# E-J408/admm-net

Measured on AMD Instinct MI355X. Metric: signals/sec (K-layer ADMM-Net forward), higher is better.
Workload: dtype f32; 1 GPU; cfg3: ADMMNet K=16 grid 16x16 (D=256, n=257) batch 65536/GPU + spectrum on 1024 atoms; batch_per_gpu=65536, global_batch=65536, K=16, D=256, n=257, natoms=1024, batch_mean_scope=global, chunk=8192, weights=torch.manual_seed(0) default init, glayer=matrix function, checked per matrix; eigensolver on the rejected matrices

## Files before the change

admm_net_amd/csrc/spectral_fused.hip:

```cpp
#include <stdio.h>
#include <stdlib.h>

#include <type_traits>

#include "common.h"
#include "rebuild_core.h"
#include "lane_reduce.h"

namespace admmnet {

constexpr int SF_THREADS = 768, SF_WAVES = 12;
constexpr int SF_PITCH = 40;
constexpr int SF_MAXM = 4;

typedef __bf16 bf16x8 __attribute__((ext_vector_type(8)));
typedef __bf16 bf16x2 __attribute__((ext_vector_type(2)));
typedef float f32x2v __attribute__((ext_vector_type(2)));
using f32x16 = __attribute__((ext_vector_type(16))) float;

__device__ __forceinline__ unsigned sf_pack_bf16(float a, float b) {
    const f32x2v p = {a, b};
    return __builtin_bit_cast(unsigned, __builtin_convertvector(p, bf16x2));
}
__device__ __forceinline__ float sf_bf16_lo(unsigned u) { return __uint_as_float(u << 16); }
// ... 19 lines not shown
#pragma unroll
    for (int q = 0; q < 4; ++q) {
        float v = 0.f;
#pragma unroll
        for (int w = 0; w < W; ++w) v += red[q * W + w];
        s[q] = v;
    }
    a = s[0]; b = s[1]; c = s[2]; d = s[3];
}

template <int W>
__device__ __forceinline__ void sf_block_sum8(float &a, float &b, float &c, float &d, float &e, float &f, float *red ) {
    const float t = sf_reduce4(a, b, c, d), u = sf_reduce4(e, f, 0.f, 0.f);
    const int lane = threadIdx.x & 63, wave = threadIdx.x >> 6;
    __syncthreads();
    if ((lane & 15) == 0) {
        red[(lane >> 4) * W + wave] = t;
        red[(4 + (lane >> 4)) * W + wave] = u;
    }
    __syncthreads();
    float s[6];
#pragma unroll
    for (int q = 0; q < 6; ++q) {
        float v = 0.f;
#pragma unroll
        for (int w = 0; w < W; ++w) v += red[q * W + w];
        s[q] = v;
    }
    a = s[0]; b = s[1]; c = s[2]; d = s[3]; e = s[4]; f = s[5];
}

struct SfCarve {
    int NP, NJ;
    float2 *X0, *X1, *Y0, *Y1, *ph, *Ob;
    float *hh, *hp, *red, *coef;
    double *sc;
    int *flags;
    float2 *part;
    unsigned short *ETre;
    unsigned short *ETim;
    __host__ __device__ static int np_of(int n) { return (n + 7) & ~7; }
    __host__ __device__ static int nj_of(int n) {
        const int D = n - 1, nt = (D + 31) >> 5;
        const int a = 32 * nt, b = (n + 7) & ~7;
        return a > b ? a : b;
    }
    __host__ __device__ static size_t bytes(int n, int W) {
        const size_t NP = np_of(n), NJ = nj_of(n);
        const size_t fixed = sizeof(float2) * 6 * NP + sizeof(float) * 2 * NP + sizeof(float) * 96 + sizeof(float) * 16 +
                             sizeof(double) * 16 + sizeof(int) * 4;
        const size_t part = sizeof(float2) * W * 2 * NP;
        const size_t slab = sizeof(unsigned short) * 2 * NJ * SF_PITCH;
        return fixed + (part > slab ? part : slab) + 64;
    }
    __device__ SfCarve(char *smem, int n) {
        NP = np_of(n);
        NJ = nj_of(n);
        sc = reinterpret_cast<double *>(smem);
        X0 = reinterpret_cast<float2 *>(sc + 16);
        X1 = X0 + NP; Y0 = X1 + NP; Y1 = Y0 + NP; ph = Y1 + NP; Ob = ph + NP;
        hh = reinterpret_cast<float *>(Ob + NP);
        hp = hh + NP;
        red = hp + NP;
        coef = red + 96;
        flags = reinterpret_cast<int *>(coef + 16);
        const int fixed = (int)(sizeof(double) * 16 + sizeof(float2) * 6 * NP + sizeof(float) * 2 * NP + sizeof(float) * 112 +
                                sizeof(int) * 4);
        char *u = smem + ((fixed + 15) & ~15);
        part = reinterpret_cast<float2 *>(u);
        ETre = reinterpret_cast<unsigned short *>(u);
        ETim = ETre + NJ * SF_PITCH;
    }
};

struct SfUpdate {
    const float *alpha;
    const float2 *phi_prev;
    const float *h_prev;
    const float *lw_prev;
    int mode;
};

__device__ __forceinline__ float2 sf_a_elem(int i, int j, int D, float2 z, float ir, float corner, float hi, float2 phj) {
    float2 a = make_float2(-ir * z.x, -ir * z.y);
    if (i < D) {
        if (i == j) a = make_float2(hi - ir * z.x, 0.f);
    } else {
        a = (j == D) ? make_float2(corner - ir * z.x, 0.f) : make_float2(phj.x - ir * z.x, -phj.y - ir * z.y);
    }
    return a;
}

template <int TPW, int W>
__global__ __launch_bounds__(64 * W, W == 12 ? 1 : 3) void sp_fused_kernel(int D, const float *__restrict__ lw, const float2 *__restrict__ phi,
                                                                 const float *__restrict__ h, float2 *Zg,
                                                                 float2 *G, float *__restrict__ rn,
                                                                 int *__restrict__ flag, int32_t *__restrict__ status, float tol,
                                                                 int iters, unsigned long long *__restrict__ ptime, SfUpdate up) {
    extern __shared__ __attribute__((aligned(16))) char smem[];
    long long t_prev = ptime ? clock64() : 0;
    auto mark = [&](int id) {
        if (ptime && threadIdx.x == 0) {
            const long long t_now = clock64();
            atomicAdd(&ptime[id], (unsigned long long)(t_now - t_prev));
            t_prev = t_now;
        }
    };
    const int n = D + 1;
    const SfCarve cv(smem, n);
    const int NP = cv.NP;
    const int64_t b = blockIdx.x;
    float2 *Z = Zg + b * (int64_t)n * n;
    const float2 *Gold = G + b * (int64_t)n * n;
    const int tid = threadIdx.x, lane = tid & 63;
    const int wave = __builtin_amdgcn_readfirstlane(tid >> 6);
    const float ir = lw[S_INV_RHO_G], corner = lw[S_CORNER_G];
    const int NT = (D + 31) >> 5, ntri = NT * (NT + 1) / 2;
    const int MM = (n + 63) >> 6;

    float pn = 0.f;
    if (tid < NP) {
        const float2 p = tid < D ? phi[b * D + tid] : make_float2(0.f, 0.f);
        cv.ph[tid] = p;
        cv.hh[tid] = tid < D ? h[b * D + tid] : 0.f;
        pn = p.x * p.x + p.y * p.y;
        if (up.mode) {
            cv.Ob[tid] = tid < D ? up.phi_prev[b * D + tid] : make_float2(0.f, 0.f);
            cv.hp[tid] = tid < D ? up.h_prev[b * D + tid] : 0.f;
        }
    }
    const float al = up.mode ? up.alpha[b] : 0.f;
    const float corner_zp = up.mode ? up.lw_prev[S_CORNER_Z] : 0.f;
    {
        float z1 = 0.f, z2 = 0.f, z3 = 0.f;
        sf_block_sum4<W>(pn, z1, z2, z3, cv.red);
    }
    const float ipn = pn > 0.f ? rsqrtf(pn) : 0.f;
    if (tid < NP) {
        const float2 p = cv.ph[tid];
        cv.X0[tid] = make_float2(tid == D ? 1.f : 0.f, 0.f);
        cv.X1[tid] = pn > 0.f ? make_float2(p.x * ipn, p.y * ipn) : make_float2(tid == 0 ? 1.f : 0.f, 0.f);
    }
    __syncthreads();

    mark(0);
    double trace = 0.0;
    float l0 = 0.f, l1 = 0.f, cf = 0.f, res0 = 0.f, res1 = 0.f;
    bool last = false;
    for (int it = 0; it < iters; ++it) {
        v2f x0[SF_MAXM], x1[SF_MAXM], c0[SF_MAXM], c1[SF_MAXM];
#pragma unroll
        for (int m = 0; m < SF_MAXM; ++m) {
            const int j = lane + 64 * m;
            const bool v = m < MM && j < n;
            x0[m] = v ? pk2(cv.X0[j]) : v2f{0.f, 0.f};
            x1[m] = v ? pk2(cv.X1[j]) : v2f{0.f, 0.f};
            c0[m] = v2f{0.f, 0.f};
            c1[m] = v2f{0.f, 0.f};
        }
        float trl = 0.f;
        auto run_pass = [&](auto updc) {
        constexpr bool UPD = decltype(updc)::value;
        float2 za[SF_MAXM], zb[SF_MAXM], zc[SF_MAXM], zd[SF_MAXM];
        float2 ga[SF_MAXM], gb[SF_MAXM], gc[SF_MAXM], gd[SF_MAXM];
        auto load_row = [&](int i, float2(&z)[SF_MAXM], float2(&g)[SF_MAXM]) {
#pragma unroll
            for (int m = 0; m < SF_MAXM; ++m) {
                const int j = lane + 64 * m;
                const bool v = i < n && j <= i;
                z[m] = (v && !(UPD && up.mode == 2)) ? Z[(int64_t)i * n + j] : make_float2(0.f, 0.f);
                if (UPD) g[m] = v ? Gold[(int64_t)i * n + j] : make_float2(0.f, 0.f);
            }
        };
        auto proc_row = [&](int i, float2(&zc)[SF_MAXM], const float2(&gq)[SF_MAXM]) {
            if (UPD) {
                const float hpi = cv.hp[i];
#pragma unroll
                for (int m = 0; m < SF_MAXM; ++m) {
                    if (64 * m <= i) {
                        const int j = lane + 64 * m;
                        if (j <= i) {
                            float2 c;
                            if (i < D) c = make_float2(i == j ? hpi : 0.f, 0.f);
                            else if (j == D) c = make_float2(corner_zp, 0.f);
                            else {
                                const float2 pp = cv.Ob[j];
                                c = make_float2(pp.x, -pp.y);
                            }
                            const float2 zn = make_float2(zc[m].x + al * (gq[m].x - c.x), zc[m].y + al * (gq[m].y - c.y));
                            zc[m] = zn;
                            Z[(int64_t)i * n + j] = zn;
                        }
                    }
                }
            }
            const v2f xi0 = pk2(cv.X0[i]), xi1 = pk2(cv.X1[i]);
            const float hi = cv.hh[i];
            v2f r0 = {0.f, 0.f}, r1 = {0.f, 0.f};
#pragma unroll
            for (int m = 0; m < SF_MAXM; ++m) {
                if (64 * m <= i) {
                    const int j = lane + 64 * m;
                    float2 a = sf_a_elem(i, j, D, zc[m], ir, corner, hi, (i == D && j < D) ? cv.ph[j] : make_float2(0.f, 0.f));
                    if (j > i) a = make_float2(0.f, 0.f);
                    if (j == i) trl += a.x;
                    const v2f av = pk2(a);
                    r0 = pk_cfma(r0, av, x0[m]);
                    r1 = pk_cfma(r1, av, x1[m]);
                    const v2f ac = (j < i) ? av : v2f{0.f, 0.f};
                    c0[m] = pk_cfma_conj(c0[m], ac, xi0);
                    c1[m] = pk_cfma_conj(c1[m], ac, xi1);
                }
            }
            if (i == 64 * SF_MAXM && lane == 0) {
                const int64_t idx = (int64_t)i * n + i;
                float2 z = (UPD && up.mode == 2) ? make_float2(0.f, 0.f) : Z[idx];
                if (UPD) {
                    const float2 g = Gold[idx];
                    z = make_float2(z.x + al * (g.x - corner_zp), z.y + al * g.y);
                    Z[idx] = z;
                }
                const float a = corner - ir * z.x;
                trl += a;
                const float2 xa = cv.X0[i], xb = cv.X1[i];
                r0.x += a * xa.x; r0.y += a * xa.y;
                r1.x += a * xb.x; r1.y += a * xb.y;
            }
            const float t = sf_reduce4(r0.x, r0.y, r1.x, r1.y);
            if ((lane & 15) == 0) {
                float *dst = reinterpret_cast<float *>((lane & 32) ? cv.Y1 : cv.Y0);
                dst[2 * i + ((lane >> 4) & 1)] = t;
            }
        };
        load_row(wave, za, ga);
        load_row(wave + W, zb, gb);
        for (int i = wave; i < n; i += 2 * W) {
            load_row(i + 2 * W, zc, gc);
            load_row(i + 3 * W, zd, gd);
            proc_row(i, za, ga);
            if (i + W < n) proc_row(i + W, zb, gb);
#pragma unroll
            for (int m = 0; m < SF_MAXM; ++m) {
                za[m] = zc[m];
                zb[m] = zd[m];
                ga[m] = gc[m];
                gb[m] = gd[m];
            }
        }
        };
        if (up.mode != 0 && it == 0) run_pass(std::true_type{});
        else run_pass(std::false_type{});
#pragma unroll
        for (int m = 0; m < SF_MAXM; ++m) {
            const int j = lane + 64 * m;
            if (m < MM && j < NP) {
                cv.part[(wave * 2 + 0) * NP + j] = make_float2(c0[m].x, c0[m].y);
                cv.part[(wave * 2 + 1) * NP + j] = make_float2(c1[m].x, c1[m].y);
            }
        }
        if (it == 0) {
            float z1 = 0.f, z2 = 0.f, z3 = 0.f;
            sf_block_sum4<W>(trl, z1, z2, z3, cv.red);
            trace = (double)trl;
        }
        __syncthreads();
        mark(1);
        float2 x0e = make_float2(0.f, 0.f), x1e = x0e, y0e = x0e, y1e = x0e;
        if (tid < n) {
            y0e = cv.Y0[tid];
            y1e = cv.Y1[tid];
#pragma unroll
            for (int w = 0; w < W; ++w) {
                if (tid >= 64 * SF_MAXM) break;
                const float2 p0 = cv.part[(w * 2 + 0) * NP + tid], p1 = cv.part[(w * 2 + 1) * NP + tid];
                y0e.x += p0.x; y0e.y += p0.y;
                y1e.x += p1.x; y1e.y += p1.y;
            }
            x0e = cv.X0[tid];
            x1e = cv.X1[tid];
        }
        float h00 = x0e.x * y0e.x + x0e.y * y0e.y, h11 = x1e.x * y1e.x + x1e.y * y1e.y;
        float h01r = x0e.x * y1e.x + x0e.y * y1e.y, h01i = x0e.x * y1e.y - x0e.y * y1e.x;
        sf_block_sum4<W>(h00, h11, h01r, h01i, cv.red);
        float ct = 1.f, st = 0.f, er = 1.f, ei = 0.f;
        {
            const float ab = sqrtf(h01r * h01r + h01i * h01i);
            const float dif = 0.5f * (h00 - h11), rad = sqrtf(dif * dif + ab * ab);
            l0 = 0.5f * (h00 + h11) - rad;
            l1 = 0.5f * (h00 + h11) + rad;
            const float vx = dif >= 0.f ? dif + rad : ab, vy = dif >= 0.f ? ab : rad - dif;
            const float nrm = sqrtf(vx * vx + vy * vy);
            if (nrm > 0.f) {
                ct = vx / nrm;
                st = vy / nrm;
            }
            if (ab > 0.f) {
                er = h01r / ab;
                ei = -h01i / ab;
            }
            cf = (float)((trace - (double)l0 - (double)l1) / (double)(n - 2));
            if (tid == 0) {
                cv.sc[0] = l0; cv.sc[1] = l1; cv.sc[2] = cf;
            }
        }
        const float2 ex1 = make_float2(er * x1e.x - ei * x1e.y, er * x1e.y + ei * x1e.x);
        const float2 ey1 = make_float2(er * y1e.x - ei * y1e.y, er * y1e.y + ei * y1e.x);
        const float2 nx0 = make_float2(-st * x0e.x + ct * ex1.x, -st * x0e.y + ct * ex1.y);
        const float2 nx1 = make_float2(ct * x0e.x + st * ex1.x, ct * x0e.y + st * ex1.y);
        const float2 ny0 = make_float2(-st * y0e.x + ct * ey1.x, -st * y0e.y + ct * ey1.y);
        const float2 ny1 = make_float2(ct * y0e.x + st * ey1.x, ct * y0e.y + st * ey1.y);
        const float2 d0 = make_float2(ny0.x - l0 * nx0.x, ny0.y - l0 * nx0.y);
        const float2 d1 = make_float2(ny1.x - l1 * nx1.x, ny1.y - l1 * nx1.y);
        float r0s = d0.x * d0.x + d0.y * d0.y, r1s = d1.x * d1.x + d1.y * d1.y;
        const float2 p0 = make_float2(ny0.x - cf * nx0.x, ny0.y - cf * nx0.y);
        const float2 p1 = make_float2(ny1.x - cf * nx1.x, ny1.y - cf * nx1.y);
        float n0 = p0.x * p0.x + p0.y * p0.y, n1 = p1.x * p1.x + p1.y * p1.y;
        float pr = p0.x * p1.x + p0.y * p1.y, pi = p0.x * p1.y - p0.y * p1.x;
        sf_block_sum8<W>(r0s, r1s, n0, n1, pr, pi, cv.red);
        res0 = sqrtf(r0s);
        res1 = sqrtf(r1s);
        last = it + 1 >= iters ||
               (it >= 1 && res0 <= 2e-6f * fabsf(l0 - cf) && res1 <= 2e-6f * fabsf(l1 - cf));
        if (!last) {
            const float in0 = n0 > 0.f ? rsqrtf(n0) : 0.f;
            const float2 q0 = make_float2(p0.x * in0, p0.y * in0);
            const float gr = pr * in0, gi = pi * in0;
            float2 q1 = make_float2(p1.x - (gr * q0.x - gi * q0.y), p1.y - (gr * q0.y + gi * q0.x));
            const float n1o = n1 - (gr * gr + gi * gi);
            const float in1 = n1o > 0.f ? rsqrtf(n1o) : 0.f;
            q1.x *= in1;
            q1.y *= in1;
            if (tid < NP) {
                cv.X0[tid] = tid < n ? q0 : make_float2(0.f, 0.f);
                cv.X1[tid] = tid < n ? q1 : make_float2(0.f, 0.f);
            }
        } else if (tid < NP) {
            cv.X0[tid] = tid < n ? nx0 : make_float2(0.f, 0.f);
            cv.X1[tid] = tid < n ? nx1 : make_float2(0.f, 0.f);
        }
        __syncthreads();
        mark(2);
        if (last) break;
    }
    const float mu0 = l0 - cf, mu1 = l1 - cf;

    int tI[TPW], tJ[TPW];
#pragma unroll
    for (int s = 0; s < TPW; ++s) tri_tile(wave * TPW + s, tI[s], tJ[s]);
    f32x16 accRe[TPW], accIm[TPW];
#pragma unroll
    for (int s = 0; s < TPW; ++s) {
#pragma unroll
        for (int q = 0; q < 16; ++q) {
            accRe[s][q] = 0.f;
            accIm[s][q] = 0.f;
        }
    }
    float2 ob = make_float2(0.f, 0.f);
    unsigned *ETre32 = reinterpret_cast<unsigned *>(cv.ETre), *ETim32 = reinterpret_cast<unsigned *>(cv.ETim);
    constexpr int P32 = SF_PITCH / 2;
    for (int idx = tid; idx < (cv.NJ - n) * P32; idx += (64 * W)) {
        ETre32[n * P32 + idx] = 0u;
        ETim32[n * P32 + idx] = 0u;
    }
    const int nslab = (n + 31) >> 5;
    for (int K = 0; K < nslab; ++K) {
        const int k0 = 32 * K;
        __syncthreads();
        int tl = tid;
        asm volatile("" : "+v"(tl));
        auto deflate = [&](float2 a, float2 vr0, float2 vc0, float2 vr1, float2 vc1, bool diag) {
            const float2 q0 = cmulc(vr0, vc0), q1 = cmulc(vr1, vc1);
            a.x -= mu0 * q0.x + mu1 * q1.x;
            a.y -= mu0 * q0.y + mu1 * q1.y;
            if (diag) {
                a.x -= cf;
                a.y = 0.f;
            }
            return a;
        };
        auto pair_of = [&](const float2 *v, int k, float2 &lo, float2 &hi) {
            const float4 t = *reinterpret_cast<const float4 *>(v + k);
            lo = make_float2(t.x, t.y);
            hi = make_float2(t.z, t.w);
        };
        {
            constexpr int RP = (64 * W) / 256, LQ = (16 + RP - 1) / RP;
            const int j = tl & 255;
            const float2 vj0 = cv.X0[j], vj1 = cv.X1[j], phj = cv.ph[j];
            constexpr int LB = 3;
// ... 98 lines not shown
                        accIm[s] = __builtin_amdgcn_mfma_f32_32x32x16_bf16(Are, Bim, accIm[s], 0, 0, 0);
                        accRe[s] = __builtin_amdgcn_mfma_f32_32x32x16_bf16(Aim, Bim, accRe[s], 0, 0, 0);
                        accIm[s] = __builtin_amdgcn_mfma_f32_32x32x16_bf16(Aim, nBre, accIm[s], 0, 0, 0);
                    }
                }
            }
        }
        mark(4);
        __syncthreads();
        if (tid < n) {
            const unsigned *dre = ETre32 + D * P32, *dim = ETim32 + D * P32;
            const unsigned *jre = ETre32 + tid * P32, *jim = ETim32 + tid * P32;
#pragma unroll 2
            for (int kp = 0; kp < 16; ++kp) {
                const unsigned ur = dre[kp], ui = dim[kp], vr = jre[kp], vi = jim[kp];
                const float ar0 = sf_bf16_lo(ur), ai0 = sf_bf16_lo(ui), br0 = sf_bf16_lo(vr), bi0 = sf_bf16_lo(vi);
                const float ar1 = sf_bf16_hi(ur), ai1 = sf_bf16_hi(ui), br1 = sf_bf16_hi(vr), bi1 = sf_bf16_hi(vi);
                {
                    asm volatile("v_fma_f32 %0, %1, %2, %0" : "+v"(ob.x) : "v"(ar0), "v"(br0));
                    asm volatile("v_fma_f32 %0, %1, %2, %0" : "+v"(ob.x) : "v"(ai0), "v"(bi0));
                    asm volatile("v_fma_f32 %0, %1, %2, %0" : "+v"(ob.x) : "v"(ar1), "v"(br1));
                    asm volatile("v_fma_f32 %0, %1, %2, %0" : "+v"(ob.x) : "v"(ai1), "v"(bi1));
                    asm volatile("v_fma_f32 %0, %1, %2, %0" : "+v"(ob.y) : "v"(ar0), "v"(bi0));
                    asm volatile("v_fma_f32 %0, -%1, %2, %0" : "+v"(ob.y) : "v"(ai0), "v"(br0));
                    asm volatile("v_fma_f32 %0, %1, %2, %0" : "+v"(ob.y) : "v"(ar1), "v"(bi1));
                    asm volatile("v_fma_f32 %0, -%1, %2, %0" : "+v"(ob.y) : "v"(ai1), "v"(br1));
                }
            }
        }
        mark(5);
    }
    __syncthreads();
    if (tid < NP) cv.Ob[tid] = tid < n ? ob : make_float2(0.f, 0.f);

    float fro = 0.f;
    {
        const int r32 = lane & 31, kh = lane >> 5;
#pragma unroll
        for (int s = 0; s < TPW; ++s) {
            if (wave * TPW + s < ntri) {
                const float wgt = tI[s] == tJ[s] ? 1.f : 2.f;
                const int gj = 32 * tJ[s] + r32;
#pragma unroll
                for (int q = 0; q < 16; ++q) {
                    const int gi = 32 * tI[s] + (q & 3) + 8 * (q >> 2) + 4 * kh;
                    if (gi < D && gj < D) fro += wgt * (accRe[s][q] * accRe[s][q] + accIm[s][q] * accIm[s][q]);
                }
            }
        }
        if (tid < n) fro += (tid < D ? 2.f : 1.f) * (ob.x * ob.x + ob.y * ob.y);
        float z1 = 0.f, z2 = 0.f, z3 = 0.f;
        sf_block_sum4<W>(fro, z1, z2, z3, cv.red);
    }
    const LayerLayout L{D};
    const float *vn = lw + L.off_vn();
    if (wave == 0) {
        const double thr = lw[S_THR];
        const double dl0 = cv.sc[0], dl1 = cv.sc[1], c = cv.sc[2];
        const double delta = sqrt(sqrt((double)fro)) * (1.0 + 0x1p-8);
        const double ts[9] = {-1.0, 0.0, 1.0, -0.75, -0.5, -0.25, 0.25, 0.5, 0.75};
        double arg = c;
        if (lane < 9) arg = c + ts[lane] * delta;
        else if (lane == 9) arg = dl0;
        else if (lane == 10) arg = dl1;
        const double fv = eig_map_f64(arg, thr, vn);
        auto bcast = [&](int src) {
            const long long bits = __builtin_bit_cast(long long, fv);
            const int lo = __builtin_amdgcn_readlane((int)(bits & 0xffffffffll), src);
            const int hi = __builtin_amdgcn_readlane((int)(bits >> 32), src);
            return __builtin_bit_cast(double, ((long long)hi << 32) | (unsigned long long)(unsigned)lo);
        };
        const double fm = bcast(0), fc = bcast(1), fp = bcast(2), f0k = bcast(9), f1k = bcast(10);
        const double a0 = fc, a1 = (fp - fm) / (2.0 * delta), a2 = (fp - 2.0 * fc + fm) / (2.0 * delta * delta);
        const double scale = fmax(fmax(fabs(fc), fmax(fabs(f0k), fabs(f1k))), 1e-6);
        double miss = 0.0;
        if (lane >= 3 && lane < 9) {
            const double t = ts[lane] * delta;
            miss = fabs(fv - (a0 + a1 * t + a2 * t * t));
        }
#pragma unroll
        for (int o = 8; o > 0; o >>= 1) miss = fmax(miss, __shfl_xor(miss, o, 64));
        if (lane == 0) {
            int why = 0;
            const double g0 = fabs(dl0 - c), g1 = fabs(dl1 - c);
            if (!(isfinite(dl0) && isfinite(dl1) && isfinite(c) && isfinite(delta) && delta > 0.0 && isfinite(miss))) why = 8;
            else if (!((double)res0 <= 1e-5 * fmax(g0, 1e-30) && (double)res1 <= 1e-5 * fmax(g1, 1e-30))) why = 1;
            else if (!(delta < 0.05 * fmin(g0, g1))) why = 2;
            else if (!(miss <= (double)tol * scale)) why = 4;
            else if (!(fabs(a2) * delta * delta <= 1e-4 * scale)) why = 16;
            cv.coef[0] = (float)(a0 - a1 * c);
            cv.coef[1] = (float)a1;
            cv.coef[2] = (float)a2;
            cv.coef[3] = (float)(f0k - a0 - a1 * (dl0 - c));
            cv.coef[4] = (float)(f1k - a0 - a1 * (dl1 - c));
            cv.flags[0] = why;
            flag[b] = why;
            if (status) {
                atomicAdd(status + (why ? 1 : 2), 1);
                if (why == 4) atomicAdd(status + 3, 1);
            }
        }
    }
    __syncthreads();
    mark(6);
    if (cv.flags[0]) return;

    const float k0c = cv.coef[0], a1f = cv.coef[1], a2f = cv.coef[2], g0f = cv.coef[3], g1f = cv.coef[4];
    const float corner_z = lw[S_CORNER_Z];
    float2 *Gb = G + b * (int64_t)n * n;
    float acc = 0.f;
    {
        const int r32 = lane & 31, kh = lane >> 5;
#pragma unroll
        for (int s = 0; s < TPW; ++s) {
            if (wave * TPW + s < ntri) {
                const int gj = 32 * tJ[s] + r32;
                const float2 vj0 = cv.X0[gj < n ? gj : 0], vj1 = cv.X1[gj < n ? gj : 0];
                constexpr int AB = 16;
#pragma unroll
                for (int qb = 0; qb < 16; qb += AB) {
                    float2 zq[AB];
#pragma unroll
                    for (int u = 0; u < AB; ++u) {
                        const int q = qb + u, gi = 32 * tI[s] + (q & 3) + 8 * (q >> 2) + 4 * kh;
                        zq[u] = (gi < D && gj <= gi) ? Z[(int64_t)gi * n + gj] : make_float2(0.f, 0.f);
                    }
#pragma unroll
                    for (int u = 0; u < AB; ++u) {
                        const int q = qb + u, gi = 32 * tI[s] + (q & 3) + 8 * (q >> 2) + 4 * kh;
                        if (gi < D && gj <= gi) {
                            const float hi = cv.hh[gi];
                            const float2 a = sf_a_elem(gi, gj, D, zq[u], ir, corner, hi, make_float2(0.f, 0.f));
                            const float2 p0 = cmulc(cv.X0[gi], vj0), p1 = cmulc(cv.X1[gi], vj1);
                            float2 g = make_float2(a1f * a.x + a2f * accRe[s][q] + g0f * p0.x + g1f * p1.x,
                                                   a1f * a.y + a2f * accIm[s][q] + g0f * p0.y + g1f * p1.y);
                            float cz = 0.f;
                            if (gi == gj) {
                                g.x += k0c;
                                g.y = 0.f;
                                cz = hi;
                            }
                            Gb[(int64_t)gi * n + gj] = g;
                            const float dr = g.x - cz;
                            acc += (gi == gj ? 1.f : 2.f) * (dr * dr + g.y * g.y);
                        }
                    }
                }
            }
        }
    }
    if (tid < n) {
        const int j = tid;
        const float2 a = sf_a_elem(D, j, D, Z[(int64_t)D * n + j], ir, corner, 0.f, cv.ph[j]);
        const float2 o = cv.Ob[j];
        const float2 p0 = cmulc(cv.X0[D], cv.X0[j]), p1 = cmulc(cv.X1[D], cv.X1[j]);
        float2 g = make_float2(a1f * a.x + a2f * o.x + g0f * p0.x + g1f * p1.x, a1f * a.y + a2f * o.y + g0f * p0.y + g1f * p1.y);
        float2 cz = make_float2(cv.ph[j].x, -cv.ph[j].y);
        if (j == D) {
            g.x += k0c;
            g.y = 0.f;
            cz = make_float2(corner_z, 0.f);
        }
        Gb[(int64_t)D * n + j] = g;
        const float dr = g.x - cz.x, di = g.y - cz.y;
        acc += (j == D ? 1.f : 2.f) * (dr * dr + di * di);
    }
    {
        float z1 = 0.f, z2 = 0.f, z3 = 0.f;
        sf_block_sum4<W>(acc, z1, z2, z3, cv.red);
    }
    if (tid == 0) rn[b] = sqrtf(acc);
    mark(7);
}

template <int TPW, int W>
static int sf_launch(int D, int64_t nb, const float *lw, const float2 *phi, const float *h, float2 *Z, float2 *G, float *rn,
                     int *flag, int32_t *status, float tol, int iters, bool timing, const SfUpdate &up, hipStream_t st) {
    const size_t lds = SfCarve::bytes(D + 1, W);
    ADMM_HIP(hipFuncSetAttribute(reinterpret_cast<const void *>(sp_fused_kernel<TPW, W>), hipFuncAttributeMaxDynamicSharedMemorySize,
                                 (int)lds));
    PhaseTimer tm;
    if (int rc = tm.begin(timing, st, 16)) return rc;
    hipLaunchKernelGGL((sp_fused_kernel<TPW, W>), dim3((unsigned)nb), dim3(64 * W), lds, st, D, lw, phi, h, Z, G, rn, flag, status,
                       tol, iters, tm.dev, up);
    ADMM_HIP(hipGetLastError());
    if (tm.dev) {
        unsigned long long hb[16];
        if (int rc = tm.end(st, hb)) return rc;
        fprintf(stderr, "[sf timing D=%d nb=%lld] cycles per workgroup: setup %.0f | matvec %.0f ritz %.0f (all passes) | stage %.0f "
                "mfma %.0f border %.0f (all slabs) | model %.0f | assemble %.0f\n", D, (long long)nb, hb[0] / (double)nb,
                hb[1] / (double)nb, hb[2] / (double)nb, (hb[3]) / (double)nb, hb[4] / (double)nb, hb[5] / (double)nb,
                hb[6] / (double)nb, hb[7] / (double)nb);
    }
    return ADMMNET_OK;
}

static_assert(SF_WAVES == 12, "spectral_waves (route.h) names the shapes 4 and 12");

int launch_spectral_fused(const Switches &sw, int D, int64_t nb, const float *lw, const float2 *phi, const float *h, float2 *Z,
                          float2 *G, float *rn, int *flag, int32_t *status, const float *alpha, const float2 *phi_prev,
                          const float *h_prev, const float *lw_prev, int update_mode, int waves, hipStream_t st) {
    const SfUpdate up{alpha, phi_prev, h_prev, lw_prev, update_mode};
    if (D < 2 || D > 256) {
        set_error("spectral: D=%d outside 2..256", D);
        return ADMMNET_E_ARG;
    }
    if (!(waves == SF_WAVES || (waves == 4 && D <= 128))) {
        set_error("spectral: %d waves per matrix at D=%d (need 12, or 4 with D <= 128)", waves, D);
        return ADMMNET_E_ARG;
    }
    const float tol = sw.spectral_tol;
    const int iters = sw.spectral_iters;
    const bool timing = sw.sf_timing;
    const int NT = (D + 31) >> 5, ntri = NT * (NT + 1) / 2;
    if (waves == 4) {
        switch ((ntri + 3) / 4) {
            case 1: return sf_launch<1, 4>(D, nb, lw, phi, h, Z, G, rn, flag, status, tol, iters, timing, up, st);
            case 2: return sf_launch<2, 4>(D, nb, lw, phi, h, Z, G, rn, flag, status, tol, iters, timing, up, st);
            default: return sf_launch<3, 4>(D, nb, lw, phi, h, Z, G, rn, flag, status, tol, iters, timing, up, st);
        }
    }
    switch ((ntri + SF_WAVES - 1) / SF_WAVES) {
        case 1: return sf_launch<1, SF_WAVES>(D, nb, lw, phi, h, Z, G, rn, flag, status, tol, iters, timing, up, st);
        case 2: return sf_launch<2, SF_WAVES>(D, nb, lw, phi, h, Z, G, rn, flag, status, tol, iters, timing, up, st);
        default: return sf_launch<3, SF_WAVES>(D, nb, lw, phi, h, Z, G, rn, flag, status, tol, iters, timing, up, st);
// ... 5 lines not shown
```

Baseline: 93960 signals/s.

## Fuse deflated-matrix staging into the last matvec pass with LDS-resident image

For the 12-wave shape, the last power/Ritz iteration now also writes a bf16 image of the deflated matrix (lower-triangle tiles plus a border strip) straight into LDS. The later MFMA spectral stage then reads that image instead of re-reading Z from global memory and re-staging it. A guard compares the predicted deflation against the final Ritz values and reruns the old path if the staged image is stale. The change adds LDS pressure (checked against a 160 KiB limit) and a serialized per-wave Y accumulation. It also adds a profiling summary script.

After: 107,200 signals/s, median of 6. 14.1% higher.

```diff
diff --git a/admm_net_amd/csrc/spectral_fused.hip b/admm_net_amd/csrc/spectral_fused.hip
--- a/admm_net_amd/csrc/spectral_fused.hip
+++ b/admm_net_amd/csrc/spectral_fused.hip
@@ -75,46 +75,70 @@
 
 struct SfCarve {
     int NP, NJ;
-    float2 *X0, *X1, *Y0, *Y1, *ph, *Ob;
+    float2 *X0, *X1, *Y0, *Y1, *ph, *Ob, *pp;
     float *hh, *hp, *red, *coef;
     double *sc;
     int *flags;
     float2 *part;
     unsigned short *ETre;
     unsigned short *ETim;
+    unsigned short *img;
+    unsigned *strip;
     __host__ __device__ static int np_of(int n) { return (n + 7) & ~7; }
     __host__ __device__ static int nj_of(int n) {
         const int D = n - 1, nt = (D + 31) >> 5;
         const int a = 32 * nt, b = (n + 7) & ~7;
         return a > b ? a : b;
     }
+    __host__ __device__ static constexpr bool resident(int W) { return W == SF_WAVES; }
+    __host__ __device__ static size_t img_bytes(int n) {
+        const size_t nt = (n - 1 + 31) >> 5;
+        return nt * (nt + 1) / 2 * 4096;
+    }
+    __host__ __device__ static size_t fixed_bytes(int n, int W) {
+        const size_t NP = np_of(n);
+        return sizeof(double) * 16 + sizeof(float2) * 6 * NP + sizeof(float) * (resident(W) ? 1 : 2) * NP + sizeof(float) * 112 +
+               sizeof(int) * 4;
+    }
     __host__ __device__ static size_t bytes(int n, int W) {
         const size_t NP = np_of(n), NJ = nj_of(n);
-        const size_t fixed = sizeof(float2) * 6 * NP + sizeof(float) * 2 * NP + sizeof(float) * 96 + sizeof(float) * 16 +
-                             sizeof(double) * 16 + sizeof(int) * 4;
         const size_t part = sizeof(float2) * W * 2 * NP;
+        if (resident(W)) {
+            const size_t a = part + sizeof(float) * 3 * NP, b = img_bytes(n) + sizeof(unsigned) * NJ;
+            return fixed_bytes(n, W) + (a > b ? a : b) + 64;
+        }
         const size_t slab = sizeof(unsigned short) * 2 * NJ * SF_PITCH;
-        return fixed + (part > slab ? part : slab) + 64;
-    }
-    __device__ SfCarve(char *smem, int n) {
+        return fixed_bytes(n, W) + (part > slab ? part : slab) + 64;
+    }
+    __device__ SfCarve(char *smem, int n, int W) {
         NP = np_of(n);
         NJ = nj_of(n);
         sc = reinterpret_cast<double *>(smem);
         X0 = reinterpret_cast<float2 *>(sc + 16);
         X1 = X0 + NP; Y0 = X1 + NP; Y1 = Y0 + NP; ph = Y1 + NP; Ob = ph + NP;
         hh = reinterpret_cast<float *>(Ob + NP);
-        hp = hh + NP;
-        red = hp + NP;
+        const bool res = resident(W);
+        hp = res ? nullptr : hh + NP;
+        pp = res ? nullptr : Ob;
+        red = res ? hh + NP : hh + 2 * NP;
         coef = red + 96;
         flags = reinterpret_cast<int *>(coef + 16);
-        const int fixed = (int)(sizeof(double) * 16 + sizeof(float2) * 6 * NP + sizeof(float) * 2 * NP + sizeof(float) * 112 +
-                                sizeof(int) * 4);
-        char *u = smem + ((fixed + 15) & ~15);
+        char *u = smem + (((int)fixed_bytes(n, W) + 15) & ~15);
         part = reinterpret_cast<float2 *>(u);
         ETre = reinterpret_cast<unsigned short *>(u);
         ETim = ETre + NJ * SF_PITCH;
+        img = reinterpret_cast<unsigned short *>(u);
+        strip = reinterpret_cast<unsigned *>(u + img_bytes(n));
+        if (res) {
+            hp = reinterpret_cast<float *>(u + sizeof(float2) * W * 2 * NP);
+            pp = reinterpret_cast<float2 *>(hp + NP);
+        }
     }
 };
+
+constexpr int SF_TILE = 2048, SF_PLANE = 1024;
+__device__ __forceinline__ int sf_img_tile(int I, int J) { return (I * (I + 1) / 2 + J) * SF_TILE; }
+__device__ __forceinline__ int sf_img_off(int r, int c) { return 32 * r + 8 * ((c >> 3) ^ ((r >> 2) & 3)) + (c & 7); }
 
 struct SfUpdate {
     const float *alpha;
@@ -150,7 +174,8 @@
         }
     };
     const int n = D + 1;
-    const SfCarve cv(smem, n);
+    const SfCarve cv(smem, n, W);
+    constexpr bool RES = SfCarve::resident(W);
     const int NP = cv.NP;
     const int64_t b = blockIdx.x;
     float2 *Z = Zg + b * (int64_t)n * n;
@@ -168,7 +193,7 @@
         cv.hh[tid] = tid < D ? h[b * D + tid] : 0.f;
         pn = p.x * p.x + p.y * p.y;
         if (up.mode) {
-            cv.Ob[tid] = tid < D ? up.phi_prev[b * D + tid] : make_float2(0.f, 0.f);
+            cv.pp[tid] = tid < D ? up.phi_prev[b * D + tid] : make_float2(0.f, 0.f);
             cv.hp[tid] = tid < D ? up.h_prev[b * D + tid] : 0.f;
         }
     }
@@ -190,30 +215,64 @@
     double trace = 0.0;
     float l0 = 0.f, l1 = 0.f, cf = 0.f, res0 = 0.f, res1 = 0.f;
     bool last = false;
-    for (int it = 0; it < iters; ++it) {
-        v2f x0[SF_MAXM], x1[SF_MAXM], c0[SF_MAXM], c1[SF_MAXM];
+    bool staged = false, padded = false;
+    float guard = 0.f;
+    float st_m0 = 0.f, st_m1 = 0.f, st_mr = 0.f, st_mi = 0.f, st_c = 0.f;
+    float pm0 = 0.f, pm1 = 0.f, pmr = 0.f, pmi = 0.f;
+    v2f x0[SF_MAXM], x1[SF_MAXM], c0[SF_MAXM], c1[SF_MAXM];
+    float trl = 0.f;
+    auto load_x = [&]() {
+        int ln = lane;
+        asm volatile("" : "+v"(ln));
 #pragma unroll
         for (int m = 0; m < SF_MAXM; ++m) {
-            const int j = lane + 64 * m;
+            const int j = ln + 64 * m;
             const bool v = m < MM && j < n;
             x0[m] = v ? pk2(cv.X0[j]) : v2f{0.f, 0.f};
             x1[m] = v ? pk2(cv.X1[j]) : v2f{0.f, 0.f};
             c0[m] = v2f{0.f, 0.f};
             c1[m] = v2f{0.f, 0.f};
         }
-        float trl = 0.f;
-        auto run_pass = [&](auto updc) {
-        constexpr bool UPD = decltype(updc)::value;
+    };
+    auto zero_pad = [&]() {
+        if (!padded && (D & 31)) {
+            unsigned *z = reinterpret_cast<unsigned *>(cv.img) + sf_img_tile(NT - 1, 0) / 2;
+            for (int idx = tid; idx < NT * (SF_TILE / 2); idx += 64 * W) z[idx] = 0u;
+            __syncthreads();
+        }
+        padded = true;
+    };
+    auto run_pass = [&](auto modec) {
+        constexpr int MODE = decltype(modec)::value;
+        constexpr bool UPD = MODE == 0, STG = MODE >= 2, MV = MODE != 3;
+        int ln = lane;
+        asm volatile("" : "+v"(ln));
         float2 za[SF_MAXM], zb[SF_MAXM], zc[SF_MAXM], zd[SF_MAXM];
         float2 ga[SF_MAXM], gb[SF_MAXM], gc[SF_MAXM], gd[SF_MAXM];
+        int lch = (ln & 31) >> 3, lfix = (ln >> 5) * SF_TILE + (ln & 7);
         auto load_row = [&](int i, float2(&z)[SF_MAXM], float2(&g)[SF_MAXM]) {
 #pragma unroll
             for (int m = 0; m < SF_MAXM; ++m) {
-                const int j = lane + 64 * m;
+                const int j = ln + 64 * m;
                 const bool v = i < n && j <= i;
                 z[m] = (v && !(UPD && up.mode == 2)) ? Z[(int64_t)i * n + j] : make_float2(0.f, 0.f);
                 if (UPD) g[m] = v ? Gold[(int64_t)i * n + j] : make_float2(0.f, 0.f);
             }
+        };
+        auto stage_w = [&](v2f xr0, v2f xr1, float2 &w0, float2 &w1) {
+            w0 = make_float2(st_m0 * xr0.x + st_mr * xr1.x + st_mi * xr1.y, st_m0 * xr0.y + st_mr * xr1.y - st_mi * xr1.x);
+            w1 = make_float2(st_m1 * xr1.x + st_mr * xr0.x - st_mi * xr0.y, st_m1 * xr1.y + st_mr * xr0.y + st_mi * xr0.x);
+        };
+        auto stage_elem = [&](float2 a, float2 w0, v2f xc0, float2 w1, v2f xc1, bool diag) {
+            const float2 q0 = cmulc(w0, make_float2(xc0.x, xc0.y));
+            const float2 q1 = cmulc(w1, make_float2(xc1.x, xc1.y));
+            a.x -= q0.x + q1.x;
+            a.y -= q0.y + q1.y;
+            if (diag) {
+                a.x -= st_c;
+                a.y = 0.f;
+            }
+            return sf_pack_bf16(a.x, a.y);
         };
         auto proc_row = [&](int i, float2(&zc)[SF_MAXM], const float2(&gq)[SF_MAXM]) {
             if (UPD) {
@@ -221,13 +280,13 @@
 #pragma unroll
                 for (int m = 0; m < SF_MAXM; ++m) {
                     if (64 * m <= i) {
-                        const int j = lane + 64 * m;
+                        const int j = ln + 64 * m;
                         if (j <= i) {
                             float2 c;
                             if (i < D) c = make_float2(i == j ? hpi : 0.f, 0.f);
                             else if (j == D) c = make_float2(corner_zp, 0.f);
                             else {
-                                const float2 pp = cv.Ob[j];
+                                const float2 pp = cv.pp[j];
                                 c = make_float2(pp.x, -pp.y);
                             }
                             const float2 zn = make_float2(zc[m].x + al * (gq[m].x - c.x), zc[m].y + al * (gq[m].y - c.y));
@@ -240,22 +299,49 @@
             const v2f xi0 = pk2(cv.X0[i]), xi1 = pk2(cv.X1[i]);
             const float hi = cv.hh[i];
             v2f r0 = {0.f, 0.f}, r1 = {0.f, 0.f};
+            float2 w0 = make_float2(0.f, 0.f), w1 = w0;
+            if (STG) {
+                stage_w(xi0, xi1, w0, w1);
+                auto uni = [](float v) { return __int_as_float(__builtin_amdgcn_readfirstlane(__float_as_int(v))); };
+                w0 = make_float2(uni(w0.x), uni(w0.y));
+                w1 = make_float2(uni(w1.x), uni(w1.y));
+            }
+            const int I = i >> 5, ir32 = i & 31;
+            const int rowoff = sf_img_tile(I, 0) + 32 * ir32 + lfix + 8 * (lch ^ ((ir32 >> 2) & 3));
 #pragma unroll
             for (int m = 0; m < SF_MAXM; ++m) {
                 if (64 * m <= i) {
-                    const int j = lane + 64 * m;
+                    const int j = ln + 64 * m;
                     float2 a = sf_a_elem(i, j, D, zc[m], ir, corner, hi, (i == D && j < D) ? cv.ph[j] : make_float2(0.f, 0.f));
                     if (j > i) a = make_float2(0.f, 0.f);
-                    if (j == i) trl += a.x;
-                    const v2f av = pk2(a);
-                    r0 = pk_cfma(r0, av, x0[m]);
-                    r1 = pk_cfma(r1, av, x1[m]);
-                    const v2f ac = (j < i) ? av : v2f{0.f, 0.f};
-                    c0[m] = pk_cfma_conj(c0[m], ac, xi0);
-                    c1[m] = pk_cfma_conj(c1[m], ac, xi1);
-                }
-            }
-            if (i == 64 * SF_MAXM && lane == 0) {
+                    if (MV) {
+                        if (j == i) trl += a.x;
+                        const v2f av = pk2(a);
+                        r0 = pk_cfma(r0, av, x0[m]);
+                        r1 = pk_cfma(r1, av, x1[m]);
+                        const v2f ac = (j < i) ? av : v2f{0.f, 0.f};
+                        c0[m] = pk_cfma_conj(c0[m], ac, xi0);
+                        c1[m] = pk_cfma_conj(c1[m], ac, xi1);
+                    }
+                    if (STG) {
+                        const unsigned e = stage_elem(a, w0, x0[m], w1, x1[m], j == i);
+                        if (i < D) {
+                            if (j <= i) {
+                                cv.img[rowoff + 2 * SF_TILE * m] = (unsigned short)e;
+                                cv.img[rowoff + 2 * SF_TILE * m + SF_PLANE] = (unsigned short)(e >> 16);
+                            }
+                            if (m == (i >> 6) && j < i && (j >> 5) == I) {
+                                const int mo = sf_img_tile(I, I) + sf_img_off(j & 31, ir32);
+                                cv.img[mo] = (unsigned short)e;
+                                cv.img[mo + SF_PLANE] = (unsigned short)((e >> 16) ^ 0x8000u);
+                            }
+                        } else if (j <= i) {
+                            cv.strip[j] = e;
+                        }
+                    }
+                }
+            }
+            if (i == 64 * SF_MAXM && ln == 0) {
                 const int64_t idx = (int64_t)i * n + i;
                 float2 z = (UPD && up.mode == 2) ? make_float2(0.f, 0.f) : Z[idx];
                 if (UPD) {
@@ -264,15 +350,24 @@
                     Z[idx] = z;
                 }
                 const float a = corner - ir * z.x;
-                trl += a;
                 const float2 xa = cv.X0[i], xb = cv.X1[i];
-                r0.x += a * xa.x; r0.y += a * xa.y;
-                r1.x += a * xb.x; r1.y += a * xb.y;
-            }
-            const float t = sf_reduce4(r0.x, r0.y, r1.x, r1.y);
-            if ((lane & 15) == 0) {
-                float *dst = reinterpret_cast<float *>((lane & 32) ? cv.Y1 : cv.Y0);
-                dst[2 * i + ((lane >> 4) & 1)] = t;
+                if (MV) {
+                    trl += a;
+                    r0.x += a * xa.x; r0.y += a * xa.y;
+                    r1.x += a * xb.x; r1.y += a * xb.y;
+                }
+                if (STG) {
+                    float2 wa, wb;
+                    stage_w(pk2(xa), pk2(xb), wa, wb);
+                    cv.strip[i] = stage_elem(make_float2(a, 0.f), wa, pk2(xa), wb, pk2(xb), true);
+                }
+            }
+            if (MV) {
+                const float t = sf_reduce4(r0.x, r0.y, r1.x, r1.y);
+                if ((ln & 15) == 0) {
+                    float *dst = reinterpret_cast<float *>((ln & 32) ? cv.Y1 : cv.Y0);
+                    dst[2 * i + ((ln >> 4) & 1)] = t;
+                }
             }
         };
         load_row(wave, za, ga);
@@ -290,9 +385,47 @@
                 gb[m] = gd[m];
             }
         }
-        };
-        if (up.mode != 0 && it == 0) run_pass(std::true_type{});
-        else run_pass(std::false_type{});
+    };
+    auto set_stage = [&](float m0, float m1, float mr, float mi, float c) {
+        st_m0 = __int_as_float(__builtin_amdgcn_readfirstlane(__float_as_int(m0)));
+        st_m1 = __int_as_float(__builtin_amdgcn_readfirstlane(__float_as_int(m1)));
+        st_mr = __int_as_float(__builtin_amdgcn_readfirstlane(__float_as_int(mr)));
+        st_mi = __int_as_float(__builtin_amdgcn_readfirstlane(__float_as_int(mi)));
+        st_c = __int_as_float(__builtin_amdgcn_readfirstlane(__float_as_int(c)));
+    };
+    for (int it = 0; it < iters; ++it) {
+        load_x();
+        trl = 0.f;
+        const bool stg = RES && it >= 1;
+        if (up.mode != 0 && it == 0) run_pass(std::integral_constant<int, 0>{});
+        else if (!stg) run_pass(std::integral_constant<int, 1>{});
+        else if constexpr (RES) {
+            zero_pad();
+            set_stage(pm0, pm1, pmr, pmi, cf);
+            run_pass(std::integral_constant<int, 2>{});
+            staged = true;
+        }
+        if (stg) {
+            __syncthreads();
+            int ln = lane;
+            asm volatile("" : "+v"(ln));
+            for (int w = 0; w < W; ++w) {
+                if (wave == w) {
+#pragma unroll
+                    for (int m = 0; m < SF_MAXM; ++m) {
+                        const int j = ln + 64 * m;
+                        if (m < MM && j < n) {
+                            float2 y0 = cv.Y0[j], y1 = cv.Y1[j];
+                            y0.x += c0[m].x; y0.y += c0[m].y;
+                            y1.x += c1[m].x; y1.y += c1[m].y;
+                            cv.Y0[j] = y0;
+                            cv.Y1[j] = y1;
+                        }
+                    }
+                }
+                __syncthreads();
+            }
+        } else {
 #pragma unroll
         for (int m = 0; m < SF_MAXM; ++m) {
             const int j = lane + 64 * m;
@@ -300,6 +433,7 @@
                 cv.part[(wave * 2 + 0) * NP + j] = make_float2(c0[m].x, c0[m].y);
                 cv.part[(wave * 2 + 1) * NP + j] = make_float2(c1[m].x, c1[m].y);
             }
+        }
         }
         if (it == 0) {
             float z1 = 0.f, z2 = 0.f, z3 = 0.f;
@@ -314,7 +448,7 @@
             y1e = cv.Y1[tid];
 #pragma unroll
             for (int w = 0; w < W; ++w) {
-                if (tid >= 64 * SF_MAXM) break;
+                if (tid >= 64 * SF_MAXM || stg) break;
                 const float2 p0 = cv.part[(w * 2 + 0) * NP + tid], p1 = cv.part[(w * 2 + 1) * NP + tid];
                 y0e.x += p0.x; y0e.y += p0.y;
                 y1e.x += p1.x; y1e.y += p1.y;
@@ -329,6 +463,7 @@
         {
             const float ab = sqrtf(h01r * h01r + h01i * h01i);
             const float dif = 0.5f * (h00 - h11), rad = sqrtf(dif * dif + ab * ab);
+            const float pc = cf;
             l0 = 0.5f * (h00 + h11) - rad;
             l1 = 0.5f * (h00 + h11) + rad;
             const float vx = dif >= 0.f ? dif + rad : ab, vy = dif >= 0.f ? ab : rad - dif;
@@ -342,6 +477,10 @@
                 ei = -h01i / ab;
             }
             cf = (float)((trace - (double)l0 - (double)l1) / (double)(n - 2));
+            {
+                const float e0 = h00 - cf - st_m0, e1 = h11 - cf - st_m1, er01 = h01r - st_mr, ei01 = h01i - st_mi;
+                guard = sqrtf(e0 * e0 + e1 * e1 + 2.f * (er01 * er01 + ei01 * ei01)) + fabsf(cf - pc);
+            }
             if (tid == 0) {
                 cv.sc[0] = l0; cv.sc[1] = l1; cv.sc[2] = cf;
             }
@@ -373,6 +512,15 @@
             const float in1 = n1o > 0.f ? rsqrtf(n1o) : 0.f;
             q1.x *= in1;
             q1.y *= in1;
+            if constexpr (RES) {
+                const float g0 = l0 - cf, g1 = l1 - cf;
+                const float i0 = in0 * in0, k0 = g0 * r0s * i0;
+                const float t = (pr * pr + pi * pi) * i0, f01 = in0 * in1 * (g1 - k0);
+                pm0 = g0 + k0;
+                pmr = f01 * pr;
+                pmi = f01 * pi;
+                pm1 = (l1 * n1 + g1 * r1s + t * (l0 + k0 - 2.f * (g0 + g1 + cf))) * (in1 * in1) - cf;
+            }
             if (tid < NP) {
                 cv.X0[tid] = tid < n ? q0 : make_float2(0.f, 0.f);
                 cv.X1[tid] = tid < n ? q1 : make_float2(0.f, 0.f);
@@ -385,20 +533,50 @@
         mark(2);
         if (last) break;
     }
+    if constexpr (RES) {
+        auto uni = [](float v) { return __int_as_float(__builtin_amdgcn_readfirstlane(__float_as_int(v))); };
+        l0 = uni(l0); l1 = uni(l1); cf = uni(cf); res0 = uni(res0); res1 = uni(res1); guard = uni(guard);
+    }
     const float mu0 = l0 - cf, mu1 = l1 - cf;
 
     int tI[TPW], tJ[TPW];
 #pragma unroll
     for (int s = 0; s < TPW; ++s) tri_tile(wave * TPW + s, tI[s], tJ[s]);
     f32x16 accRe[TPW], accIm[TPW];
-#pragma unroll
-    for (int s = 0; s < TPW; ++s) {
-#pragma unroll
-        for (int q = 0; q < 16; ++q) {
-            accRe[s][q] = 0.f;
-            accIm[s][q] = 0.f;
-        }
-    }
+    auto zero_acc = [&]() {
+#pragma unroll
+        for (int s = 0; s < TPW; ++s) {
+#pragma unroll
+            for (int q = 0; q < 16; ++q) {
+                accRe[s][q] = 0.f;
+                accIm[s][q] = 0.f;
+            }
+        }
+    };
+    auto frob = [&](float2 o) {
+        float fro = 0.f;
+        int r32 = lane & 31, kh = lane >> 5;
+        asm volatile("" : "+v"(r32), "+v"(kh));
+#pragma unroll
+        for (int s = 0; s < TPW; ++s) {
+            if (wave * TPW + s < ntri) {
+                const float wgt = tI[s] == tJ[s] ? 1.f : 2.f;
+                const int gj = 32 * tJ[s] + r32;
+#pragma unroll
+                for (int q = 0; q < 16; ++q) {
+                    const int gi = 32 * tI[s] + (q & 3) + 8 * (q >> 2) + 4 * kh;
+                    if (gi < D && gj < D) fro += wgt * (accRe[s][q] * accRe[s][q] + accIm[s][q] * accIm[s][q]);
+                }
+            }
+        }
+        if (tid < n) fro += (tid < D ? 2.f : 1.f) * (o.x * o.x + o.y * o.y);
+        float z1 = 0.f, z2 = 0.f, z3 = 0.f;
+        sf_block_sum4<W>(fro, z1, z2, z3, cv.red);
+        return fro;
+    };
+    float fro = 0.f;
+    if constexpr (!RES) {
+    zero_acc();
     float2 ob = make_float2(0.f, 0.f);
     unsigned *ETre32 = reinterpret_cast<unsigned *>(cv.ETre), *ETim32 = reinterpret_cast<unsigned *>(cv.ETim);
     constexpr int P32 = SF_PITCH / 2;
@@ -563,26 +741,180 @@
     }
     __syncthreads();
     if (tid < NP) cv.Ob[tid] = tid < n ? ob : make_float2(0.f, 0.f);
-
-    float fro = 0.f;
-    {
-        const int r32 = lane & 31, kh = lane >> 5;
-#pragma unroll
-        for (int s = 0; s < TPW; ++s) {
-            if (wave * TPW + s < ntri) {
-                const float wgt = tI[s] == tJ[s] ? 1.f : 2.f;
-                const int gj = 32 * tJ[s] + r32;
-#pragma unroll
-                for (int q = 0; q < 16; ++q) {
-                    const int gi = 32 * tI[s] + (q & 3) + 8 * (q >> 2) + 4 * kh;
-                    if (gi < D && gj < D) fro += wgt * (accRe[s][q] * accRe[s][q] + accIm[s][q] * accIm[s][q]);
-                }
-            }
-        }
-        if (tid < n) fro += (tid < D ? 2.f : 1.f) * (ob.x * ob.x + ob.y * ob.y);
-        float z1 = 0.f, z2 = 0.f, z3 = 0.f;
-        sf_block_sum4<W>(fro, z1, z2, z3, cv.red);
-    }
+    fro = frob(ob);
+    } else {
+    bool spec = staged;
+    auto attempt = [&]() -> bool {
+        if (!staged) {
+            zero_pad();
+            set_stage(mu0, mu1, 0.f, 0.f, cf);
+            load_x();
+            run_pass(std::integral_constant<int, 3>{});
+            staged = true;
+            __syncthreads();
+        }
+        mark(3);
+        zero_acc();
+        typedef short s16x4 __attribute__((ext_vector_type(4)));
+        typedef __attribute__((address_space(3))) s16x4 *lds_s16x4;
+        auto rd_row = [&](int o) { return *reinterpret_cast<const uint4 *>(cv.img + o); };
+        auto rd_tr = [&](int o0, int o1) {
+            const uint2 lo = __builtin_bit_cast(uint2, __builtin_amdgcn_ds_read_tr16_b64_v4i16((lds_s16x4)(cv.img + o0)));
+            const uint2 hi = __builtin_bit_cast(uint2, __builtin_amdgcn_ds_read_tr16_b64_v4i16((lds_s16x4)(cv.img + o1)));
+            return make_uint4(lo.x, lo.y, hi.x, hi.y);
+        };
+        {
+            int r32 = lane & 31, kh = lane >> 5;
+            asm volatile("" : "+v"(r32), "+v"(kh));
+            const int rsw = (r32 >> 2) & 3;
+            const int row_o[2] = {32 * r32 + 8 * (kh ^ rsw), 32 * r32 + 8 * ((2 + kh) ^ rsw)};
+            const int tq = (lane & 15) >> 2, tp = lane & 3, tc = 2 * ((lane >> 4) & 1) + (tp >> 1);
+            const int tr_o0 = 32 * (8 * kh + tq) + 8 * (tc ^ ((2 * kh) & 3)) + 4 * (tp & 1);
+            const int tr_o1 = 32 * (8 * kh + 4 + tq) + 8 * (tc ^ ((2 * kh + 1) & 3)) + 4 * (tp & 1);
+            constexpr unsigned SGN = 0x80008000u;
+            for (int K = 0; K < NT; ++K) {
+#pragma unroll
+                for (int ks = 0; ks < 2; ++ks) {
+                    uint4 are = make_uint4(0, 0, 0, 0), aim = are;
+                    unsigned ma = 0u;
+#pragma unroll
+                    for (int s = 0; s < TPW; ++s) {
+                        if (wave * TPW + s < ntri) {
+                            const int I = tI[s], J = tJ[s];
+                            if (s == 0 || tI[s] != tI[s - 1]) {
+                                if (K <= I) {
+                                    const int base = sf_img_tile(I, K) + row_o[ks];
+                                    are = rd_row(base);
+                                    aim = rd_row(base + SF_PLANE);
+                                    ma = 0u;
+                                } else {
+                                    const int base = sf_img_tile(K, I) + 512 * ks;
+                                    are = rd_tr(base + tr_o0, base + tr_o1);
+                                    aim = rd_tr(base + SF_PLANE + tr_o0, base + SF_PLANE + tr_o1);
+                                    ma = SGN;
+                                }
+                            }
+                            uint4 bre, bim;
+                            unsigned mb;
+                            if (K >= J) {
+                                const int base = sf_img_tile(K, J) + 512 * ks;
+                                bre = rd_tr(base + tr_o0, base + tr_o1);
+                                bim = rd_tr(base + SF_PLANE + tr_o0, base + SF_PLANE + tr_o1);
+                                mb = 0u;
+                            } else {
+                                const int base = sf_img_tile(J, K) + row_o[ks];
+                                bre = rd_row(base);
+                                bim = rd_row(base + SF_PLANE);
+                                mb = SGN;
+                            }
+                            const unsigned mn = ma ^ mb ^ SGN;
+                            const uint4 bi1 = make_uint4(bim.x ^ mb, bim.y ^ mb, bim.z ^ mb, bim.w ^ mb);
+                            const uint4 bi2 = make_uint4(bim.x ^ mn, bim.y ^ mn, bim.z ^ mn, bim.w ^ mn);
+                            const uint4 br2 = make_uint4(bre.x ^ ma, bre.y ^ ma, bre.z ^ ma, bre.w ^ ma);
+                            const bf16x8 Are = __builtin_bit_cast(bf16x8, are), Aim = __builtin_bit_cast(bf16x8, aim);
+                            const bf16x8 Bre = __builtin_bit_cast(bf16x8, bre), Bi1 = __builtin_bit_cast(bf16x8, bi1);
+                            const bf16x8 Bi2 = __builtin_bit_cast(bf16x8, bi2), Br2 = __builtin_bit_cast(bf16x8, br2);
+                            accRe[s] = __builtin_amdgcn_mfma_f32_32x32x16_bf16(Are, Bre, accRe[s], 0, 0, 0);
+                            accIm[s] = __builtin_amdgcn_mfma_f32_32x32x16_bf16(Are, Bi1, accIm[s], 0, 0, 0);
+                            accRe[s] = __builtin_amdgcn_mfma_f32_32x32x16_bf16(Aim, Bi2, accRe[s], 0, 0, 0);
+                            accIm[s] = __builtin_amdgcn_mfma_f32_32x32x16_bf16(Aim, Br2, accIm[s], 0, 0, 0);
+                        }
+                    }
+                }
+            }
+        }
+        mark(4);
+        __syncthreads();
+        {
+            int r32 = lane & 31, kh = lane >> 5;
+            asm volatile("" : "+v"(r32), "+v"(kh));
+#pragma unroll
+            for (int s = 0; s < TPW; ++s) {
+                if (wave * TPW + s < ntri) {
+                    const unsigned uj = cv.strip[32 * tJ[s] + r32];
+                    const float ejr = sf_bf16_lo(uj), eji = sf_bf16_hi(uj);
+#pragma unroll
+                    for (int qq = 0; qq < 4; ++qq) {
+                        const int gi = 32 * tI[s] + 8 * qq + 4 * kh;
+                        const uint4 u4 = *reinterpret_cast<const uint4 *>(cv.strip + gi);
+                        const unsigned ui[4] = {u4.x, u4.y, u4.z, u4.w};
+#pragma unroll
+                        for (int e = 0; e < 4; ++e) {
+                            const float eir = sf_bf16_lo(ui[e]), eii = sf_bf16_hi(ui[e]);
+                            accRe[s][4 * qq + e] += eir * ejr + eii * eji;
+                            accIm[s][4 * qq + e] += eir * eji - eii * ejr;
+                        }
+                    }
+                }
+            }
+        }
+        {
+            int tl = tid;
+            asm volatile("" : "+v"(tl));
+            constexpr int NG = (64 * W) / 256;
+            const int g = tl >> 8, j = tl & 255, J = j >> 5, jr = j & 31;
+            float2 ob = make_float2(0.f, 0.f);
+            if (j < D) {
+                for (int K = g; K < NT; K += NG) {
+                    const int kend = D - 32 * K < 32 ? D - 32 * K : 32;
+                    const bool low = K >= J;
+                    const int base = low ? sf_img_tile(K, J) : sf_img_tile(J, K);
+                    const unsigned isg = low ? 0u : 0x80000000u;
+                    for (int kk = 0; kk < kend; ++kk) {
+                        const int o = base + (low ? sf_img_off(kk, jr) : sf_img_off(jr, kk));
+                        const unsigned ue = cv.strip[32 * K + kk];
+                        const float ar = sf_bf16_lo(ue), ai = sf_bf16_hi(ue);
+                        const float br = __uint_as_float((unsigned)cv.img[o] << 16);
+                        const float bi = __uint_as_float(((unsigned)cv.img[o + SF_PLANE] << 16) ^ isg);
+                        asm volatile("v_fma_f32 %0, %1, %2, %0" : "+v"(ob.x) : "v"(ar), "v"(br));
+                        asm volatile("v_fma_f32 %0, -%1, %2, %0" : "+v"(ob.x) : "v"(ai), "v"(bi));
+                        asm volatile("v_fma_f32 %0, %1, %2, %0" : "+v"(ob.y) : "v"(ar), "v"(bi));
+                        asm volatile("v_fma_f32 %0, %1, %2, %0" : "+v"(ob.y) : "v"(ai), "v"(br));
+                    }
+                }
+            }
+            if (g == 1 && j < D) cv.Y0[j] = ob;
+            if (g == 2 && j < D) cv.Y1[j] = ob;
+            __syncthreads();
+            const float eD = sf_bf16_lo(cv.strip[D]);
+            if (g == 0) {
+                if (j < D) {
+                    const float2 p1 = cv.Y0[j], p2 = cv.Y1[j];
+                    const unsigned uj = cv.strip[j];
+                    ob.x = (ob.x + p1.x) + p2.x + eD * sf_bf16_lo(uj);
+                    ob.y = (ob.y + p1.y) + p2.y + eD * sf_bf16_hi(uj);
+                    cv.Ob[j] = ob;
+                } else if (j > D && j < NP) {
+                    cv.Ob[j] = make_float2(0.f, 0.f);
+                }
+            } else if (wave == W - 1) {
+                float sq = 0.f;
+                for (int k = lane; k < D; k += 64) {
+                    const unsigned ue = cv.strip[k];
+                    const float ar = sf_bf16_lo(ue), ai = sf_bf16_hi(ue);
+                    sq += ar * ar + ai * ai;
+                }
+                sq = wave_sum(sq);
+                if (lane == 0) {
+                    cv.Ob[D] = make_float2(sq + eD * eD, 0.f);
+                    for (int jj = 256; jj < NP; ++jj)
+                        if (jj != D) cv.Ob[jj] = make_float2(0.f, 0.f);
+                }
+            }
+            __syncthreads();
+        }
+        fro = frob(tid < n ? cv.Ob[tid] : make_float2(0.f, 0.f));
+        mark(5);
+        if (spec && guard > 0x1p-5f * sqrtf(sqrtf(fro))) {
+            spec = false;
+            staged = false;
+            return true;
+        }
+        return false;
+    };
+    if (attempt()) attempt();
+    }
+
     const LayerLayout L{D};
     const float *vn = lw + L.off_vn();
     if (wave == 0) {
@@ -641,7 +973,8 @@
     float2 *Gb = G + b * (int64_t)n * n;
     float acc = 0.f;
     {
-        const int r32 = lane & 31, kh = lane >> 5;
+        int r32 = lane & 31, kh = lane >> 5;
+        asm volatile("" : "+v"(r32), "+v"(kh));
 #pragma unroll
         for (int s = 0; s < TPW; ++s) {
             if (wave * TPW + s < ntri) {
@@ -708,6 +1041,10 @@
 static int sf_launch(int D, int64_t nb, const float *lw, const float2 *phi, const float *h, float2 *Z, float2 *G, float *rn,
                      int *flag, int32_t *status, float tol, int iters, bool timing, const SfUpdate &up, hipStream_t st) {
     const size_t lds = SfCarve::bytes(D + 1, W);
+    if (lds > 160 * 1024) {
+        set_error("spectral: %zu bytes of LDS at D=%d, %d waves (a workgroup has 163840)", lds, D, W);
+        return ADMMNET_E_ARG;
+    }
     ADMM_HIP(hipFuncSetAttribute(reinterpret_cast<const void *>(sp_fused_kernel<TPW, W>), hipFuncAttributeMaxDynamicSharedMemorySize,
                                  (int)lds));
     PhaseTimer tm;
@@ -718,10 +1055,10 @@
     if (tm.dev) {
         unsigned long long hb[16];
         if (int rc = tm.end(st, hb)) return rc;
-        fprintf(stderr, "[sf timing D=%d nb=%lld] cycles per workgroup: setup %.0f | matvec %.0f ritz %.0f (all passes) | stage %.0f "
-                "mfma %.0f border %.0f (all slabs) | model %.0f | assemble %.0f\n", D, (long long)nb, hb[0] / (double)nb,
-                hb[1] / (double)nb, hb[2] / (double)nb, (hb[3]) / (double)nb, hb[4] / (double)nb, hb[5] / (double)nb,
-                hb[6] / (double)nb, hb[7] / (double)nb);
+        fprintf(stderr, "[sf timing D=%d nb=%lld] cycles per workgroup: setup %.0f | matvec%s %.0f ritz %.0f (all passes) | stage %.0f "
+                "mfma %.0f border %.0f | model %.0f | assemble %.0f\n", D, (long long)nb, hb[0] / (double)nb,
+                SfCarve::resident(W) ? "+stage" : "", hb[1] / (double)nb, hb[2] / (double)nb, (hb[3]) / (double)nb,
+                hb[4] / (double)nb, hb[5] / (double)nb, hb[6] / (double)nb, hb[7] / (double)nb);
     }
     return ADMMNET_OK;
 }
diff --git a/profiles/r10/summarize.py b/profiles/r10/summarize.py
--- /dev/null
+++ b/profiles/r10/summarize.py
@@ -0,0 +1,30 @@
+import csv
+import glob
+import os
+import sys
+from collections import defaultdict
+
+
+def main(root, per=0):
+    for f in sorted(glob.glob(os.path.join(root, "**", "*kernel_stats.csv"), recursive=True)):
+        rows = list(csv.DictReader(open(f)))
+        total = sum(float(r["TotalDurationNs"]) for r in rows)
+        for r in sorted(rows, key=lambda r: -float(r["TotalDurationNs"]))[:8]:
+            print(f"{r['Name'][:60]:60s} calls {int(r['Calls']):6d} mean {float(r['AverageNs']) / 1e6:8.3f} ms "
+                  f"share {100 * float(r['TotalDurationNs']) / total:5.1f} %")
+    for f in sorted(glob.glob(os.path.join(root, "**", "*counter_collection.csv"), recursive=True)):
+        acc = defaultdict(lambda: [0.0, 0])
+        for r in csv.DictReader(open(f)):
+            if "sp_fused_kernel" in r["Kernel_Name"]:
+                a = acc[(r["Kernel_Name"][:40], r["Counter_Name"])]
+                a[0] += float(r["Counter_Value"])
+                a[1] += 1
+        for (k, c), (v, cnt) in sorted(acc.items()):
+            line = f"{k:40s} {c}: mean per dispatch {v / cnt:.1f} over {cnt} dispatches"
+            if per:
+                line += f", per matrix {v / cnt / per:.4f}"
+            print(line)
+
+
+if __name__ == "__main__":
+    main(sys.argv[1], int(sys.argv[2]) if len(sys.argv) > 2 else 0)
```
